# GuoYi0/alphaFive

Hardware: AMD Instinct MI355X
Metric: self-play moves/sec (11x11, 500 sims/move) (higher is better)
Workload: dtype f32 (fp16x2 split operands: 3 fp16 MFMA products per MAC, fp32 accumulate)

## Files before the change

alphafive_amd/csrc/af_engine.hip:

```cpp

#include <hip/hip_runtime.h>
#include <stdint.h>
#include <stdio.h>
#include <stdlib.h>
#include <string.h>

#include <type_traits>
#include <vector>

#include "af_engine.h"
#include "af_noise.h"

typedef unsigned long long u64;

enum { PH_IDLE = 0, PH_MOVE_START = 1, PH_SEARCH = 2, PH_MOVE_DONE = 3, PH_ERROR = 4, PH_DESCENT = 5  };
enum { CT_SIMS = 0, CT_SELECTS, CT_EXPANDS, CT_TERMINALS, CT_PLIES, CT_EPISODES, CT_LSUM, CT_LEXP,
       CT_GC, CT_GC_SCANNED, CT_YIELDS, CT_STALLS, CT_N };
enum { HIST_WORK = 0, HIST_TIME = 64, HIST_MAXTIME = 96, HIST_N = 97 };

struct EngineParams {
    int G, S, C, goal, sims, upper, training, mode, node_cap, max_ply, budget, budget_hard;
    uint32_t hash_mask;
    double init_temp, tau_decay, tau_decay_r, alpha, c_puct;
    float c_puct32;
    uint32_t k0, seed_hi, first_game_id;
    u64 colmask[4], boardmask[4];
    int32_t *phase, *pending, *sims_left, *ply, *root_last, *nodes, *nfree, *depth, *leaf_last, *leaf_slot, *status, *random_a;
    int32_t *action, *has_policy, *visits;
    float* policy;
    u64 *root, *leaf;
    double* tau;
    uint32_t *episode, *sel, *plyctr;
    int32_t *path_node, *path_cell;
    uint32_t* hash;
    u64* node_key;
    int32_t* node_sum;
    int32_t* free_idx;
    int32_t* edge_n;
    float *edge_w, *edge_p;
    int32_t* edge_c;
    double* edge_w64;
    int32_t w64;
    uint32_t *ep_seq, *ep_popped;
    int32_t* ep_len;
    float* ep_final;
    u64* rec_key;
    float* rec_policy;
    int32_t *rec_visits, *rec_last, *rec_action;
    u64* counters;
    u64* progress;
    u64* hist;
    u64* memo_key;
    float* memo_pv;
    float* memo_val;
    u64* memo_lock;
    u64* memo_stats;
    uint32_t memo_bucket_mask;
    int memo_max_stones;
    uint32_t memo_epoch;
    int memo_budget;
};
enum { MEMO_SERIAL = 0, MEMO_PROBES, MEMO_HITS, MEMO_INSERTS, MEMO_REPLACED, MEMO_N };

__device__ __forceinline__ uint32_t rfl32(uint32_t x) { return (uint32_t)__builtin_amdgcn_readfirstlane((int)x); }
__device__ __forceinline__ int rfli(int x) { return __builtin_amdgcn_readfirstlane(x); }
__device__ __forceinline__ u64 rfl64(u64 x) {
    return ((u64)rfl32((uint32_t)(x >> 32)) << 32) | (u64)rfl32((uint32_t)x);
}
__device__ __forceinline__ float rflf(float x) { return __int_as_float(rfli(__float_as_int(x))); }
template <int CTRL, int ROWS = 0xF>
__device__ __forceinline__ int dpp_i(int v) { return __builtin_amdgcn_update_dpp(v, v, CTRL, ROWS, 0xF, false); }
__device__ __forceinline__ int wave_max_i32(int v) {
    int o;
    o = dpp_i<0xB1>(v); v = o > v ? o : v;
    o = dpp_i<0x4E>(v); v = o > v ? o : v;
    o = dpp_i<0x141>(v); v = o > v ? o : v;
    o = dpp_i<0x140>(v); v = o > v ? o : v;
    o = dpp_i<0x142, 0xA>(v); v = o > v ? o : v;
    o = dpp_i<0x143, 0xC>(v); v = o > v ? o : v;
    return __builtin_amdgcn_readlane(v, 63);
}
__device__ __forceinline__ float wave_max_f32(float v) {
    float o;
    o = __int_as_float(dpp_i<0xB1>(__float_as_int(v))); v = o > v ? o : v;
    o = __int_as_float(dpp_i<0x4E>(__float_as_int(v))); v = o > v ? o : v;
    o = __int_as_float(dpp_i<0x141>(__float_as_int(v))); v = o > v ? o : v;
    o = __int_as_float(dpp_i<0x140>(__float_as_int(v))); v = o > v ? o : v;
    o = __int_as_float(dpp_i<0x142, 0xA>(__float_as_int(v))); v = o > v ? o : v;
    o = __int_as_float(dpp_i<0x143, 0xC>(__float_as_int(v))); v = o > v ? o : v;
    return __int_as_float(__builtin_amdgcn_readlane(__float_as_int(v), 63));
}


template <int CTRL>
__device__ __forceinline__ double dpp_f64(double v) {
    const int lo = __double2loint(v), hi = __double2hiint(v);
    return __hiloint2double(__builtin_amdgcn_update_dpp(hi, hi, CTRL, 0xF, 0xF, false), __builtin_amdgcn_update_dpp(lo, lo, CTRL, 0xF, 0xF, false));
}
__device__ __forceinline__ double wave_sum_f64_tree(double acc) {
    {
        const int lo = __double2loint(acc), hi = __double2hiint(acc);
        const auto a = __builtin_amdgcn_permlane32_swap(lo, lo, false, false), b = __builtin_amdgcn_permlane32_swap(hi, hi, false, false);
        acc = __hiloint2double(b[0], a[0]) + __hiloint2double(b[1], a[1]);
    }
    {
        const int lo = __double2loint(acc), hi = __double2hiint(acc);
        const auto a = __builtin_amdgcn_permlane16_swap(lo, lo, false, false), b = __builtin_amdgcn_permlane16_swap(hi, hi, false, false);
        acc = __hiloint2double(b[0], a[0]) + __hiloint2double(b[1], a[1]);
    }
    acc = acc + dpp_f64<0x128>(acc);
    acc = acc + dpp_f64<0x124>(acc);
    acc = acc + dpp_f64<0x4E>(acc);
    acc = acc + dpp_f64<0xB1>(acc);
// ... 199 lines not shown
    return h & P.memo_bucket_mask;
}
template <int KW>
__device__ __forceinline__ u64 memo_word(const EngineParams& P, const u64* mine, const u64* theirs, int last, int w) {
    const u64 kw = key_word<KW>(mine, theirs, w);
    return w == 2 * KW ? (((u64)P.memo_epoch << 32) | (u64)(uint32_t)(last + 1)) : kw;
}
template <int KW>
__device__ __forceinline__ int memo_probe(const EngineParams& P, uint32_t bucket, const u64* mine, const u64* theirs, int last, int lane,
                                          uint32_t* empty_ways) {
    constexpr int MK = 4 * KW;
    const int w = lane & (MK - 1);
    const u64 expect = memo_word<KW>(P, mine, theirs, last, w);
    u64 have = expect;
    if (lane < 4 * MK) have = P.memo_key[(size_t)bucket * (4 * MK) + lane];
    const u64 bad = __ballot(have != expect);
    const u64 blank = __ballot(lane < 4 * MK && w == 2 * KW && (uint32_t)(have >> 32) != P.memo_epoch);
    uint32_t em = 0;
    int hit = -1;
#pragma unroll
    for (int v = 3; v >= 0; --v) {
        const u64 wm = (MK == 16 ? 0xffffull : 0xffull) << (v * MK);
        if ((bad & wm) == 0ull) hit = (int)bucket * 4 + v;
        if (blank & wm) em |= 1u << v;
    }
    *empty_ways = em;
    return hit;
}


__device__ float pairwise_block(const float* a, int n) {
    if (n < 8) {
        float r = 0.0f;
        for (int i = 0; i < n; ++i) r = r + a[i];
        return r;
    }
    float r0 = a[0], r1 = a[1], r2 = a[2], r3 = a[3], r4 = a[4], r5 = a[5], r6 = a[6], r7 = a[7];
    int i;
    for (i = 8; i < n - (n % 8); i += 8) {
        r0 = r0 + a[i]; r1 = r1 + a[i + 1]; r2 = r2 + a[i + 2]; r3 = r3 + a[i + 3];
        r4 = r4 + a[i + 4]; r5 = r5 + a[i + 5]; r6 = r6 + a[i + 6]; r7 = r7 + a[i + 7];
    }
    float res = ((r0 + r1) + (r2 + r3)) + ((r4 + r5) + (r6 + r7));
    for (; i < n; ++i) res = res + a[i];
    return res;
}
__device__ float pairwise_sum(const float* a, int n) {
    if (n <= 128) return pairwise_block(a, n);
    int n2 = n / 2;
    n2 -= n2 % 8;
    return pairwise_block(a, n2) + pairwise_block(a + n2, n - n2);
}

#ifndef AF_TICK_MIN_WAVES
#define AF_TICK_MIN_WAVES 4
#endif
#ifdef AF_TICK_TIMING
__device__ unsigned long long g_tick_cycles[8192][13];
#define TK_T(var) const unsigned long long var = __builtin_readcyclecounter()
#define TK_ACC(slot, a, b) tk[slot] += (b) - (a)
#else
#define TK_T(var)
#define TK_ACC(slot, a, b)
#endif

template <int KW, bool W64, bool MEMO = false>
__global__ __launch_bounds__(64, AF_TICK_MIN_WAVES) void af_tick_kernel(EngineParams P, const float* __restrict__ policy_in,
                                                     const float* __restrict__ value_in, float* __restrict__ planes_out) {
    constexpr int CP = 64 * KW;
    __shared__ float s_pv[CP];
    __shared__ double s_cdf[CP];
    const int g = blockIdx.x;
    const int lane = threadIdx.x;
    const int C = P.C, NCAP = P.node_cap;
    if constexpr (MEMO) {
        if (g == 0 && lane == 0) atomicAdd(reinterpret_cast<unsigned long long*>(&P.memo_stats[MEMO_SERIAL]), 1ull);
    }

    int phase = rfli(P.phase[g]);
    if (phase == PH_IDLE || phase == PH_MOVE_DONE || phase == PH_ERROR) return;
    const u64 t_start = wall_clock64();
#ifdef AF_TICK_TIMING
    unsigned long long tk[13] = {0, 0, 0, 0, 0, 0, 0, 0, 0, 0, 0, 0, 0};
#endif
    TK_T(tk_entry);

    u64 root_m[KW], root_t[KW];
#pragma unroll
    for (int k = 0; k < KW; ++k) {
        root_m[k] = rfl64(P.root[(size_t)g * 2 * KW + k]);
        root_t[k] = rfl64(P.root[(size_t)g * 2 * KW + KW + k]);
    }
    int root_last = rfli(P.root_last[g]);
    int sims_left = rfli(P.sims_left[g]);
    int ply = rfli(P.ply[g]);
    int nodes = rfli(P.nodes[g]);
    int nfree = rfli(P.nfree[g]);
    double tau = P.tau[g];
    uint32_t episode = rfl32(P.episode[g]);
    uint32_t sel = rfl32(P.sel[g]);
    uint32_t plyctr = rfl32(P.plyctr[g]);
    const int random_a = rfli(P.random_a[g]);
    const uint32_t inv_s16 = (65536u + (uint32_t)P.S - 1u) / (uint32_t)P.S;
    const uint32_t k0 = P.k0, k1 = P.seed_hi + (P.first_game_id + (uint32_t)g);
    uint32_t ct[CT_N];
#pragma unroll
    for (int i = 0; i < CT_N; ++i) ct[i] = 0;
    int err = 0;

    u64* const nkeys = P.node_key + (size_t)g * NCAP * (2 * KW);
    int32_t* const nsum = P.node_sum + (size_t)g * NCAP;
    int32_t* const fre = P.free_idx + (size_t)g * NCAP;
    int32_t* const en = P.edge_n + (size_t)g * NCAP * CP;
    constexpr bool w64 = W64;
    float* const ew = P.edge_w + (w64 ? (size_t)0 : (size_t)g * NCAP * CP);
    double* const ew64 = P.edge_w64 + (w64 ? (size_t)g * NCAP * CP : (size_t)0);
    float* const ep = P.edge_p + (size_t)g * NCAP * CP;
    int32_t* const ec = P.edge_c + (size_t)g * NCAP * CP;
    uint32_t* const slots = P.hash + (size_t)g * (P.hash_mask + 1);
    int32_t* const pnode = P.path_node + (size_t)g * CP;
    int32_t* const pcell = P.path_cell + (size_t)g * CP;

    auto backup = [&](int depth, float v, int is_f32) {
        for (int d = lane; d < depth; d += 64) {
            const size_t off = (size_t)pnode[d] * CP + pcell[d];
            const float vv = ((depth - d) & 1) ? -v : v;
            const int32_t raw = en[off];
            if (w64) {
                en[off] = raw + 1;
                ew64[off] = ew64[off] + (double)vv;
            } else {
                en[off] = (raw + 1) | (is_f32 ? (int32_t)0x80000000 : 0);
                ew[off] = ew[off] + vv;
            }
        }
        __syncthreads();
    };

    TK_T(tk_loaded);
    TK_ACC(0, tk_entry, tk_loaded);
    u64 lm[KW], lt[KW];
    int c_depth = 0;
    uint32_t c_slot = 0;
    const float* c_pol = policy_in + (size_t)g * C;
    const float* c_val = value_in + g;
    bool have_eval = rfli(P.pending[g]) != 0;
    if (have_eval) {
#pragma unroll
        for (int k = 0; k < KW; ++k) {
            lm[k] = rfl64(P.leaf[(size_t)g * 2 * KW + k]);
            lt[k] = rfl64(P.leaf[(size_t)g * 2 * KW + KW + k]);
        }
        c_depth = rfli(P.depth[g]);
        c_slot = rfl32((uint32_t)P.leaf_slot[g]);
    }
    int status = AF_STATUS_IDLE;
    bool parked = false;
    int work = 0;
    uint32_t memo_probes = 0, memo_hits = 0;
  for (;;) {
    if (have_eval) {
        have_eval = false;
        u64 legal[KW];
#pragma unroll
        for (int k = 0; k < KW; ++k) legal[k] = ~(lm[k] | lt[k]) & P.boardmask[k];
        const int depth = c_depth;
        const uint32_t slot = c_slot;
        float pk[KW];
#pragma unroll
        for (int k = 0; k < KW; ++k) {
            const int c = lane + 64 * k;
            pk[k] = ((legal[k] >> lane) & 1ull) ? c_pol[c] : 0.0f;
        }
#pragma unroll
        for (int k = 0; k < KW; ++k) s_pv[lane + 64 * k] = pk[k];
        __syncthreads();
        float s = 0.0f;
#pragma unroll
        for (int i = 0; i < CP; i += 4) {
            const float4 v4 = *reinterpret_cast<const float4*>(&s_pv[i]);
            s = s + v4.x; s = s + v4.y; s = s + v4.z; s = s + v4.w;
        }
        s = rflf(s);
        if (!((double)s >= 1e-5)) s = (float)1e-5;
        if ((nfree == 0 && nodes >= NCAP) || slot == 0xffffffffu) {
            err = AF_ERR_NODE_CAP;
        } else {
            int idx;
            if (nfree > 0) idx = rfli(fre[--nfree]); else idx = nodes++;
            if (lane < 2 * KW) nkeys[(size_t)idx * 2 * KW + lane] = key_word<KW>(lm, lt, lane);
            if (lane == 0) {
                nsum[idx] = 0; slots[slot] = (uint32_t)idx + 1u;
                if (depth > 0) ec[(size_t)pnode[depth - 1] * CP + pcell[depth - 1]] = idx + 1;
            }
#pragma unroll
            for (int k = 0; k < KW; ++k) {
                const size_t off = (size_t)idx * CP + lane + 64 * k;
                en[off] = 0;
                ec[off] = 0;
                if (w64) ew64[off] = 0.0; else ew[off] = 0.0f;
                ep[off] = ((legal[k] >> lane) & 1ull) ? pk[k] / s : 0.0f;
            }
            __syncthreads();
            backup(depth, rflf(*c_val), 1);
            ct[CT_EXPANDS]++;
            ct[CT_LEXP] += (uint32_t)bb_count<KW>(legal);
        }
        ct[CT_SIMS]++;
        sims_left--;
    }

    TK_T(tk_consumed);
    TK_ACC(1, tk_loaded, tk_consumed);
    while (!parked && !err && !(MEMO && have_eval)) {
        TK_T(tk_iter);
        if (work >= ((MEMO && memo_hits) ? P.memo_budget : P.budget) && phase != PH_DESCENT) { status = AF_STATUS_YIELD; parked = true; ct[CT_YIELDS]++; break; }
        if (phase == PH_MOVE_START) {
            if (P.mode == AF_MODE_SELFPLAY && ply == 0 && rfl32(P.ep_seq[g]) - rfl32(P.ep_popped[g]) >= 2u) {
                status = AF_STATUS_YIELD; parked = true; ct[CT_STALLS]++;
                break;
            }
            bool collected = false;
            if (nodes - nfree + P.sims + 2 > NCAP && nodes > 0) {
                for (uint32_t s_ = lane; s_ <= P.hash_mask; s_ += 64) slots[s_] = 0;
                __syncthreads();
                const int rc = bb_count<KW>(root_m) + bb_count<KW>(root_t);
                int nf = 0;
                for (int base = 0; base < nodes; base += 64) {
                    const int i = base + lane;
                    const bool valid = i < nodes;
                    bool keep = false;
                    if (valid && nsum[i] >= 0) {
                        u64 nm[KW], nt[KW];
#pragma unroll
                        for (int k = 0; k < KW; ++k) { nm[k] = nkeys[(size_t)i * 2 * KW + k]; nt[k] = nkeys[(size_t)i * 2 * KW + KW + k]; }
                        const int nc = bb_count<KW>(nm) + bb_count<KW>(nt);
                        keep = true;
#pragma unroll
                        for (int k = 0; k < KW; ++k) {
                            const u64 a = ((nc ^ rc) & 1) ? nt[k] : nm[k];
                            const u64 b = ((nc ^ rc) & 1) ? nm[k] : nt[k];
                            keep = keep && ((a & root_m[k]) == root_m[k]) && ((b & root_t[k]) == root_t[k]);
                        }
                        if (keep) {
                            uint32_t h = key_hash<KW>(nm, nt);
                            for (;;) {
                                h &= P.hash_mask;
                                if (atomicCAS(&slots[h], 0u, (uint32_t)i + 1u) == 0u) break;
                                ++h;
                            }
                        } else {
                            nsum[i] = -1;
                        }
                    }
                    const u64 dm = __ballot(valid && !keep);
                    if (valid && !keep) fre[nf + __popcll(dm & ((1ull << lane) - 1ull))] = i;
                    nf += __popcll(dm);
                }
                nfree = nf;
                __syncthreads();
                __threadfence();
                ct[CT_GC]++; ct[CT_GC_SCANNED] += (uint32_t)nodes;
                collected = true;
            }
            uint32_t slot;
            const int ridx = tree_lookup<KW>(P, g, root_m, root_t, lane, &slot);
// ... 88 lines not shown
            }
#pragma unroll
            for (int k = 0; k < KW; ++k) {
                P.policy[(size_t)g * CP + lane + 64 * k] = pol[k];
                P.visits[(size_t)g * CP + lane + 64 * k] = nv[k] < 0 ? 0 : nv[k];
            }
            if (lane == 0) { P.action[g] = action; P.has_policy[g] = has_policy; }

            if (P.mode == AF_MODE_EXTERNAL) {
                phase = PH_MOVE_DONE;
                status = AF_STATUS_MOVE_DONE;
                parked = true;
                break;
            }
            if (ply >= P.max_ply) { err = AF_ERR_STATE; break; }
            const uint32_t seq = rfl32(P.ep_seq[g]);
            const size_t rslot = ((size_t)g * 2 + (seq & 1u)) * P.max_ply + ply;
            if (lane < 2 * KW) P.rec_key[rslot * 2 * KW + lane] = key_word<KW>(root_m, root_t, lane);
#pragma unroll
            for (int k = 0; k < KW; ++k) {
                const int c = lane + 64 * k;
                if (c < C) { P.rec_policy[rslot * C + c] = pol[k]; P.rec_visits[rslot * C + c] = nv[k] < 0 ? 0 : nv[k]; }
            }
            if (lane == 0) { P.rec_last[rslot] = root_last; P.rec_action[rslot] = action; }
            {
                u64 nm[KW], nt[KW];
#pragma unroll
                for (int k = 0; k < KW; ++k) { nm[k] = root_t[k]; nt[k] = root_m[k]; }
                bb_set<KW>(nt, action);
#pragma unroll
                for (int k = 0; k < KW; ++k) { root_m[k] = nm[k]; root_t[k] = nt[k]; }
            }
            root_last = action;
            ++ply;
            float fv;
            if (terminal_test<KW>(P, root_m, root_t, &fv)) {
                if (seq - rfl32(P.ep_popped[g]) >= 2u) { err = AF_ERR_EP_OVERRUN; break; }
                if (lane == 0) {
                    P.ep_len[(size_t)g * 2 + (seq & 1u)] = ply;
                    P.ep_final[(size_t)g * 2 + (seq & 1u)] = fv;
                    P.ep_seq[g] = seq + 1u;
                }
                ct[CT_EPISODES]++;
                if (lane == 0) atomicAdd(&P.progress[1], 1ull);
                for (uint32_t s_ = lane; s_ <= P.hash_mask; s_ += 64) slots[s_] = 0;
                __syncthreads();
                nodes = 0; nfree = 0;
#pragma unroll
                for (int k = 0; k < KW; ++k) { root_m[k] = 0; root_t[k] = 0; }
                root_last = -1;
                ply = 0;
                tau = P.init_temp;
                episode += 1; sel = 0; plyctr = 0;
            }
            phase = PH_MOVE_START;
            continue;
        }

        TK_T(tk_sim);
        TK_ACC(2, tk_iter, tk_sim);
        u64 cm[KW], ctb[KW];
        int last, depth;
        if (phase == PH_DESCENT) {
#pragma unroll
            for (int k = 0; k < KW; ++k) {
                cm[k] = rfl64(P.leaf[(size_t)g * 2 * KW + k]);
                ctb[k] = rfl64(P.leaf[(size_t)g * 2 * KW + KW + k]);
            }
            last = rfli(P.leaf_last[g]); depth = rfli(P.depth[g]);
            phase = PH_SEARCH;
        } else {
#pragma unroll
            for (int k = 0; k < KW; ++k) { cm[k] = root_m[k]; ctb[k] = root_t[k]; }
            last = root_last; depth = 0;
        }
        int hint = 0, pidx = -1, pcl = 0;
        typedef typename std::conditional<W64, double, float>::type wrow_t;
        int32_t r_raw[KW], r_c[KW];
        float r_p[KW];
        wrow_t r_w[KW];
        int32_t r_sum = 0;
        bool r_have = false;
        for (;;) {
            TK_T(tk_a);
            float tv;
            bool term;
            if (depth == 0)
                term = P.mode == AF_MODE_EXTERNAL ? (bool)terminal_test<KW, false>(P, cm, ctb, &tv) : false;
            else
                term = (depth > 0 && P.goal <= 8) ? (bool)terminal_through_last<KW>(P, cm, ctb, last, inv_s16, lane, &tv)
                                                                       : (bool)terminal_test<KW, true>(P, cm, ctb, &tv);
            if (term) {
                backup(depth, tv, 0);
                ct[CT_TERMINALS]++; ct[CT_SIMS]++;
                sims_left--;
                break;
            }
            uint32_t slot = 0xffffffffu;
            int idx;
            if (hint) {
                idx = hint - 1;
            } else {
                idx = tree_lookup<KW>(P, g, cm, ctb, lane, &slot);
                if (idx >= 0 && pidx >= 0 && lane == 0) ec[(size_t)pidx * CP + pcl] = idx + 1;
            }
            if (idx < 0) {
                if constexpr (MEMO) {
                    if (slot != 0xffffffffu && bb_count<KW>(cm) + bb_count<KW>(ctb) <= P.memo_max_stones) {
                        uint32_t unused;
                        const int me = memo_probe<KW>(P, memo_bucket<KW>(P, cm, ctb, last), cm, ctb, last, lane, &unused);
                        ++memo_probes;
                        if (me >= 0) {
                            ++memo_hits;
#pragma unroll
                            for (int k = 0; k < KW; ++k) { lm[k] = cm[k]; lt[k] = ctb[k]; }
                            c_depth = depth; c_slot = slot;
                            c_pol = P.memo_pv + (size_t)me * CP;
                            c_val = P.memo_val + me;
                            have_eval = true;
                            break;
                        }
                    }
                }
                if (lane < 2 * KW) P.leaf[(size_t)g * 2 * KW + lane] = key_word<KW>(cm, ctb, lane);
                if (lane == 0) { P.depth[g] = depth; P.leaf_last[g] = last; P.leaf_slot[g] = (int32_t)slot; }
                float* out = planes_out + (size_t)g * 3 * C;
#pragma unroll
                for (int k = 0; k < KW; ++k) {
                    const int c = lane + 64 * k;
                    if (c < C) {
                        out[c] = ((cm[k] >> lane) & 1ull) ? 1.0f : 0.0f;
                        out[C + c] = ((ctb[k] >> lane) & 1ull) ? 1.0f : 0.0f;
                        out[2 * C + c] = c == last ? 1.0f : 0.0f;
                    }
                }
                status = AF_STATUS_NEED_EVAL;
                parked = true;
                break;
            }
            if (work >= P.budget_hard) {
                if (lane < 2 * KW) P.leaf[(size_t)g * 2 * KW + lane] = key_word<KW>(cm, ctb, lane);
                if (lane == 0) { P.depth[g] = depth; P.leaf_last[g] = last; }
                phase = PH_DESCENT; status = AF_STATUS_YIELD; parked = true; ct[CT_YIELDS]++;
                break;
            }
            TK_T(tk_b);
            TK_ACC(3, tk_a, tk_b);
            const bool is_root = depth == 0;
            u64 legal[KW];
#pragma unroll
            for (int k = 0; k < KW; ++k) legal[k] = ~(cm[k] | ctb[k]) & P.boardmask[k];
            if (!r_have) {
                r_sum = nsum[idx];
#pragma unroll
                for (int k = 0; k < KW; ++k) {
                    const size_t off = (size_t)idx * CP + lane + 64 * k;
                    r_raw[k] = en[off];
                    r_c[k] = ec[off];
                    if constexpr (W64) r_w[k] = ew64[off]; else r_w[k] = ew[off];
                    r_p[k] = ep[off];
                }
            }
            r_have = false;
            const int sum_n = rfli(r_sum) + 1;
            if (lane == 0) nsum[idx] = sum_n;
            const uint32_t sel_id = sel++;
            int nn[KW];
            float pp[KW];
            wrow_t ww[KW];
            bool ff[KW];
            int32_t cc[KW];
#pragma unroll
            for (int k = 0; k < KW; ++k) {
                nn[k] = r_raw[k] & 0x7fffffff;
                ff[k] = r_raw[k] < 0;
                cc[k] = r_c[k];
                ww[k] = r_w[k];
                pp[k] = r_p[k];
            }
            double dd[KW];
            if (P.training) {
#ifdef AF_TICK_TIMING
                int tk_myit = 0;
#endif
                {
                    const float a_ = (float)P.alpha, inv_a = 1.0f / a_, one_m_a = 1.0f - a_;
                    uint32_t todo = 0;
#pragma unroll
                    for (int k = 0; k < KW; ++k) { dd[k] = 0.0; todo |= ((legal[k] >> lane) & 1ull) ? (1u << k) : 0u; }
                    af_u32x4 rk[KW];
                    uint32_t pend = 0;
#pragma unroll
                    for (int k = 0; k < KW; ++k) {
                        rk[k] = af_philox4x32(sel_id, episode, (AF_STREAM_GAMMA << 24) | (uint32_t)(lane + 64 * k), 0u, k0, k1);
                        float X;
                        const int ok = af_gamma_round(a_, inv_a, one_m_a, rk[k].v[0], rk[k].v[1], &X);
                        const bool lg = (todo >> k) & 1u;
                        dd[k] = (lg && ok) ? (double)X : 0.0;
                        pend |= (lg && !ok) ? (1u << k) : 0u;
                        if (KW > 2 && (k & 1)) __builtin_amdgcn_sched_barrier(0);
                    }
#ifdef AF_TICK_TIMING
                    ++tk_myit;
#endif
                    todo = pend;
                    {
                    uint32_t it = 1;
                    af_u32x4 r = rk[0];
#pragma unroll
                    for (int q = 1; q < KW; ++q) if (!(todo & ((1u << q) - 1u))) r = rk[q];
                    while (todo) {
#ifdef AF_TICK_TIMING
                        ++tk_myit;
#endif
                        const int k = __builtin_ctz(todo);
                        if ((it & 1u) == 0u) r = af_philox4x32(sel_id, episode, (AF_STREAM_GAMMA << 24) | (uint32_t)(lane + 64 * k), it >> 1, k0, k1);
                        const uint32_t wu = (it & 1u) ? r.v[2] : r.v[0], wv = (it & 1u) ? r.v[3] : r.v[1];
                        float X;
                        const int ok = af_gamma_round(a_, inv_a, one_m_a, wu, wv, &X);
                        if (ok || it == 0xFFFFu) {
                            const double Xd = ok ? (double)X : 0.0;
#pragma unroll
                            for (int q = 0; q < KW; ++q) dd[q] = q == k ? Xd : dd[q];
                            todo &= todo - 1u;
                            it = 1;
#pragma unroll
                            for (int q = 1; q < KW; ++q) if (todo && !(todo & ((1u << q) - 1u))) r = rk[q];
                        } else {
                            ++it;
                        }
                    }
                    }
                }
#ifdef AF_TICK_TIMING
                tk[12] += (unsigned long long)wave_max_i32(tk_myit);
#endif
                TK_T(tk_n1);
                TK_ACC(8, tk_b, tk_n1);
                double acc = 0.0;
#pragma unroll
                for (int k = 0; k < KW; ++k) acc = k == 0 ? dd[0] : acc + dd[k];
                acc = wave_sum_f64_tree(acc);
                if (acc == 0.0) {
                    int cnt = 0;
#pragma unroll
                    for (int k = 0; k < KW; ++k) cnt += __popcll(legal[k]);
                    const double u = 1.0 / (double)cnt;
#pragma unroll
                    for (int k = 0; k < KW; ++k) dd[k] = ((legal[k] >> lane) & 1ull) ? u : 0.0;
                } else {
                    const double inv = 1.0 / acc;
#pragma unroll
                    for (int k = 0; k < KW; ++k) dd[k] = dd[k] * inv;
                }
                TK_T(tk_n1e);
                TK_ACC(9, tk_n1, tk_n1e);
            }
            TK_T(tk_n2);
            const double sq = sqrt((double)(sum_n + 1));
            float sc[KW];
            float mx = -3.0e38f;
#pragma unroll
            for (int k = 0; k < KW; ++k) {
                const bool lg = (legal[k] >> lane) & 1ull;
                double q64;
                if (nn[k] == 0) q64 = 0.0;
                else if (!W64 && ff[k]) q64 = (double)((float)ww[k] / (float)nn[k]);
                else q64 = (double)ww[k] / (double)nn[k];
                double t;
                if (P.training) {
                    double p_;
                    if (is_root) p_ = (double)(0.75f * pp[k]) + 0.25 * dd[k];
                    else p_ = (double)(0.9f * pp[k]) + 0.1 * dd[k];
                    t = ((P.c_puct * p_) * sq) / (double)(1 + nn[k]);
                } else {
                    t = ((double)(P.c_puct32 * pp[k]) * sq) / (double)(1 + nn[k]);
                }
                sc[k] = lg ? (float)(q64 + t) : -3.0e38f;
                mx = sc[k] > mx ? sc[k] : mx;
            }
            TK_T(tk_n3);
            TK_ACC(10, tk_n2, tk_n3);
            int cell = -1;
            if (is_root && P.training) {
                u64 cand[KW];
#pragma unroll
                for (int k = 0; k < KW; ++k) cand[k] = __ballot(((legal[k] >> lane) & 1ull) && nn[k] == 0);
                int m = bb_count<KW>(cand);
                if (m == 0) {
#pragma unroll
                    for (int k = 0; k < KW; ++k) cand[k] = __ballot(((legal[k] >> lane) & 1ull) && nn[k] == 1);
                    m = bb_count<KW>(cand);
                }
                if (m > 0) cell = bb_select_wave<KW>(cand, (int)af_pick((uint32_t)m, sel_id, episode, AF_STREAM_PICK, k0, k1), lane);
            }
            if (cell < 0) {
                mx = wave_max_f32(mx);
                u64 cand[KW];
#pragma unroll
                for (int k = 0; k < KW; ++k) cand[k] = __ballot(((legal[k] >> lane) & 1ull) && sc[k] == mx);
                const int m = bb_count<KW>(cand);
                cell = bb_select_wave<KW>(cand, (int)af_pick((uint32_t)m, sel_id, episode, AF_STREAM_PICK, k0, k1), lane);
            }
            cell = rfli(cell);
            hint = 0;
#pragma unroll
            for (int k = 0; k < KW; ++k) { const int t_ = __builtin_amdgcn_readlane(cc[k], cell & 63); if ((cell >> 6) == k) hint = t_; }
            hint = rfli(hint);
            pidx = idx; pcl = cell;
            if (hint) {
                const int ci = hint - 1;
                r_sum = nsum[ci];
#pragma unroll
                for (int k = 0; k < KW; ++k) {
                    const size_t off = (size_t)ci * CP + lane + 64 * k;
                    r_raw[k] = en[off];
                    r_c[k] = ec[off];
                    if constexpr (W64) r_w[k] = ew64[off]; else r_w[k] = ew[off];
                    r_p[k] = ep[off];
                }
                r_have = true;
            }
            ++work;
            ct[CT_SELECTS]++;
            ct[CT_LSUM] += (uint32_t)bb_count<KW>(legal);
            if (lane == 0) { pnode[depth] = idx; pcell[depth] = cell; }
            ++depth;
            {
                u64 nm[KW], nt[KW];
#pragma unroll
                for (int k = 0; k < KW; ++k) { nm[k] = ctb[k]; nt[k] = cm[k]; }
                bb_set<KW>(nt, cell);
#pragma unroll
                for (int k = 0; k < KW; ++k) { cm[k] = nm[k]; ctb[k] = nt[k]; }
            }
            last = cell;
            __syncthreads();
            TK_T(tk_c);
            TK_ACC(4, tk_b, tk_c);
            TK_ACC(11, tk_n3, tk_c);
#ifdef AF_TICK_TIMING
            tk[7] += 1;
#endif
        }
    }
    if (!MEMO || !have_eval) break;
  }
    TK_T(tk_parked);
    if constexpr (MEMO) {
        if (lane == 0 && memo_probes) {
            atomicAdd(reinterpret_cast<unsigned long long*>(&P.memo_stats[MEMO_PROBES]), (unsigned long long)memo_probes);
            if (memo_hits) atomicAdd(reinterpret_cast<unsigned long long*>(&P.memo_stats[MEMO_HITS]), (unsigned long long)memo_hits);
        }
    }

    if (err) { phase = PH_ERROR; status = err; }
    if (lane < 2 * KW) P.root[(size_t)g * 2 * KW + lane] = key_word<KW>(root_m, root_t, lane);
    if (lane == 0) {
        P.phase[g] = phase;
        P.pending[g] = status == AF_STATUS_NEED_EVAL ? 1 : 0;
        P.root_last[g] = root_last;
        P.sims_left[g] = sims_left;
        P.ply[g] = ply;
        P.nodes[g] = nodes;
        P.nfree[g] = nfree;
        P.tau[g] = tau;
        P.episode[g] = episode;
        P.sel[g] = sel;
        P.plyctr[g] = plyctr;
        P.status[g] = status;
        for (int i = 0; i < CT_N; ++i)
            if (ct[i]) atomicAdd(reinterpret_cast<unsigned long long*>(&P.counters[(size_t)g * CT_N + i]), (unsigned long long)ct[i]);
        const u64 dt = wall_clock64() - t_start;
        atomicAdd(&P.hist[HIST_WORK + (work < 63 ? work : 63)], 1ull);
        const u64 tb = dt / 800ull;
        atomicAdd(&P.hist[HIST_TIME + (tb < 31ull ? tb : 31ull)], 1ull);
        atomicMax(&P.hist[HIST_MAXTIME], dt);
    }
#ifdef AF_TICK_TIMING
    {
        TK_T(tk_end);
        tk[5] = tk_end - tk_parked;
        tk[6] = tk_end - tk_entry;
        if (lane == 0 && g < 8192) for (int q = 0; q < 13; ++q) g_tick_cycles[g][q] = tk[q];
    }
#endif
}

__global__ __launch_bounds__(1024) void af_pack_scan(EngineParams P, int max_eps, int max_plies, int32_t* __restrict__ out) {
    __shared__ int s_e[1024], s_p[1024];
    __shared__ int s_cut;
    const int t = threadIdx.x;
    int base_e = 0, base_p = 0;
    int32_t* meta = out + 4;
    int32_t* fin = out + 4 + (size_t)max_eps * 4;
    if (t == 0) s_cut = 0x7fffffff;
    __syncthreads();
    for (int g0 = 0; g0 < P.G; g0 += 1024) {
        const int g = g0 + t;
        int ne = 0, T0 = 0, T1 = 0;
        uint32_t pop = 0;
        if (g < P.G) {
            pop = P.ep_popped[g];
            ne = (int)(P.ep_seq[g] - pop);
            if (ne >= 1) T0 = P.ep_len[(size_t)g * 2 + (pop & 1u)];
            if (ne >= 2) T1 = P.ep_len[(size_t)g * 2 + ((pop + 1u) & 1u)];
        }
        s_e[t] = ne; s_p[t] = T0 + T1;
        __syncthreads();
        for (int off = 1; off < 1024; off <<= 1) {
            const int ve = t >= off ? s_e[t - off] : 0, vp = t >= off ? s_p[t - off] : 0;
            __syncthreads();
            s_e[t] += ve; s_p[t] += vp;
            __syncthreads();
        }
        const int e_excl = base_e + s_e[t] - ne, p_excl = base_p + s_p[t] - (T0 + T1);
        int fit = 0;
        if (ne >= 1 && e_excl + 1 <= max_eps && p_excl + T0 <= max_plies) {
            fit = 1;
            if (ne >= 2 && e_excl + 2 <= max_eps && p_excl + T0 + T1 <= max_plies) fit = 2;
        }
        if (g < P.G && fit < ne) atomicMin(&s_cut, g);
        __syncthreads();
        const int cut = s_cut;
        if (g < P.G && g <= cut && fit > 0) {
            for (int k = 0; k < fit; ++k) {
                const uint32_t seq = pop + (uint32_t)k;
                const int idx = e_excl + k;
                meta[idx * 4 + 0] = g; meta[idx * 4 + 1] = (int32_t)seq;
                meta[idx * 4 + 2] = k == 0 ? T0 : T1; meta[idx * 4 + 3] = p_excl + (k == 0 ? 0 : T0);
                fin[idx] = __float_as_int(P.ep_final[(size_t)g * 2 + (seq & 1u)]);
            }
            P.ep_popped[g] = pop + (uint32_t)fit;
        }
        __syncthreads();
        if (cut != 0x7fffffff) {
            if (g == cut) {
// ... 151 lines not shown
        case AF_ERR_STATE: return "engine state error";
        default: return "unknown error";
    }
}

int af_engine_create(const af_config* cfg, int32_t num_games, int32_t device, int32_t mode, int32_t training,
                     uint64_t seed, uint32_t first_game_id, int32_t node_cap, af_engine** out) {
    if (!cfg || !out || num_games < 1) return AF_ERR_ARG;
    const int S = cfg->board_size, C = S * S;
    if (S < 2 || C > 256 || cfg->goal < 2 || cfg->goal > S || cfg->simulation_per_step < 1) return AF_ERR_ARG;
    const int value_f64 = (mode & AF_MODE_VALUE_F64) ? 1 : 0;
    mode &= ~AF_MODE_VALUE_F64;
    if (mode != AF_MODE_SELFPLAY && mode != AF_MODE_EXTERNAL) return AF_ERR_ARG;
    if (!(cfg->dirichlet_alpha > 0.0 && cfg->dirichlet_alpha < 1.0)) return AF_ERR_ARG;
    if (cfg->upper_simulation_per_step < 1 || !(cfg->c_puct >= 0.0)) return AF_ERR_ARG;
    HIP_OK(hipSetDevice(device));
    af_engine* e = new af_engine();
    e->device = device;
    e->KW = C <= 128 ? 2 : 4;
    const int KW = e->KW, CP = 64 * KW;
    EngineParams& P = e->P;
    memset(&P, 0, sizeof(P));
    P.G = num_games; P.S = S; P.C = C; P.goal = cfg->goal;
    P.sims = cfg->simulation_per_step; P.upper = cfg->upper_simulation_per_step;
    P.training = training ? 1 : 0; P.mode = mode; P.max_ply = C; P.w64 = value_f64;
    P.budget = AF_DEFAULT_TICK_BUDGET; P.budget_hard = AF_DEFAULT_TICK_BUDGET_HARD;
    if (const char* b = getenv("AF_TICK_BUDGET")) { const int v = atoi(b); if (v > 0) P.budget = v; }
    if (const char* b = getenv("AF_TICK_BUDGET_HARD")) { const int v = atoi(b); if (v > 0) P.budget_hard = v; }
    if (P.budget_hard < P.budget) P.budget_hard = P.budget;
    if (node_cap <= 0) node_cap = mode == AF_MODE_SELFPLAY ? 4 * P.sims + 64 : 32768;
    if (node_cap < P.sims + 8) node_cap = P.sims + 8;
    P.node_cap = node_cap;
    uint32_t hcap = 64;
    while (hcap < 2u * (uint32_t)node_cap) hcap <<= 1;
    P.hash_mask = hcap - 1;
    P.init_temp = cfg->init_temp; P.tau_decay = cfg->tau_decay_rate; P.tau_decay_r = cfg->tau_decay_rate_r;
    P.alpha = cfg->dirichlet_alpha; P.c_puct = cfg->c_puct; P.c_puct32 = (float)cfg->c_puct;
    P.k0 = af_key0(seed); P.seed_hi = (uint32_t)(seed >> 32); P.first_game_id = first_game_id;
    for (int c = 0; c < C; ++c) {
        P.boardmask[c >> 6] |= 1ull << (c & 63);
        if (c % S <= S - cfg->goal) P.colmask[c >> 6] |= 1ull << (c & 63);
    }
    const size_t G = num_games;
    int rc = AF_OK;
#define A(p, n) if (rc == AF_OK) rc = dalloc(e, &P.p, (n))
    A(phase, G); A(pending, G); A(sims_left, G); A(ply, G); A(root_last, G); A(nodes, G); A(nfree, G); A(depth, G);
    A(leaf_last, G); A(leaf_slot, G); A(status, G); A(random_a, G); A(action, G); A(has_policy, G);
    A(visits, G * CP); A(policy, G * CP); A(root, G * 2 * KW); A(leaf, G * 2 * KW); A(tau, G);
    A(episode, G); A(sel, G); A(plyctr, G); A(path_node, G * CP); A(path_cell, G * CP);
    A(hash, G * hcap); A(node_key, G * node_cap * 2 * KW); A(node_sum, G * node_cap); A(free_idx, G * node_cap);
    A(edge_n, G * node_cap * CP); A(edge_p, G * node_cap * CP); A(edge_c, G * node_cap * CP);
    if (value_f64) { A(edge_w64, G * node_cap * CP); A(edge_w, 64); } else { A(edge_w, G * node_cap * CP); A(edge_w64, 8); }
    A(ep_seq, G); A(ep_popped, G); A(counters, G * CT_N); A(progress, 2); A(hist, HIST_N);
    if (mode == AF_MODE_SELFPLAY) {
        const size_t R = G * 2 * P.max_ply;
        A(ep_len, G * 2); A(ep_final, G * 2); A(rec_key, R * 2 * KW); A(rec_policy, R * C); A(rec_visits, R * C);
        A(rec_last, R); A(rec_action, R);
    }
#undef A
    if (rc != AF_OK) { af_engine_destroy(e); return rc; }
    std::vector<int32_t> ph(G, mode == AF_MODE_SELFPLAY ? PH_MOVE_START : PH_IDLE), rl(G, -1);
    std::vector<double> tau(G, cfg->init_temp);
    HIP_OK(hipMemcpy(P.phase, ph.data(), G * 4, hipMemcpyHostToDevice));
    HIP_OK(hipMemcpy(P.root_last, rl.data(), G * 4, hipMemcpyHostToDevice));
    HIP_OK(hipMemcpy(P.tau, tau.data(), G * 8, hipMemcpyHostToDevice));
    e->h_i32.resize(G); e->h_i32b.resize(G); e->h_ct.resize(G * CT_N);
    *out = e;
    return AF_OK;
}

void af_engine_destroy(af_engine* e) {
    if (!e) return;
    (void)hipSetDevice(e->device);
    for (void* p : e->allocs) (void)hipFree(p);
    if (e->pack_dev) (void)hipFree(e->pack_dev);
    if (e->stage_dev) (void)hipFree(e->stage_dev);
    delete e;
}

int32_t af_engine_num_games(const af_engine* e) { return e->P.G; }
int32_t af_engine_cells(const af_engine* e) { return e->P.C; }
int32_t af_engine_key_words(const af_engine* e) { return 2 * e->KW; }
int32_t af_engine_max_plies(const af_engine* e) { return e->P.max_ply; }

int af_engine_tick(af_engine* e, void* stream, const float* policy_dev, const float* value_dev, float* planes_dev) {
    if (!e || !planes_dev) return AF_ERR_ARG;
    hipStream_t st = (hipStream_t)stream;
#define AF_TICK(KW_, W_, M_) hipLaunchKernelGGL((af_tick_kernel<KW_, W_, M_>), dim3(e->P.G), dim3(64), 0, st, e->P, policy_dev, value_dev, planes_dev)
    if (e->memo) {
        if (e->KW == 2) { if (e->P.w64) AF_TICK(2, true, true); else AF_TICK(2, false, true); }
        else { if (e->P.w64) AF_TICK(4, true, true); else AF_TICK(4, false, true); }
    } else {
        if (e->KW == 2) { if (e->P.w64) AF_TICK(2, true, false); else AF_TICK(2, false, false); }
        else { if (e->P.w64) AF_TICK(4, true, false); else AF_TICK(4, false, false); }
    }
#undef AF_TICK
    HIP_OK(hipGetLastError());
    return AF_OK;
}

int af_engine_memo_enable(af_engine* e, int32_t log2_buckets, int32_t max_stones) {
    if (!e || e->memo || log2_buckets < 4 || log2_buckets > 28 || max_stones < 0) return AF_ERR_ARG;
    HIP_OK(hipSetDevice(e->device));
    EngineParams& P = e->P;
    const size_t NE = (size_t)4 << log2_buckets, CP = 64 * (size_t)e->KW, MK = 4 * (size_t)e->KW;
    int rc = AF_OK;
    if (rc == AF_OK) rc = dalloc(e, &P.memo_key, NE * MK);
    if (rc == AF_OK) rc = dalloc(e, &P.memo_pv, NE * CP);
    if (rc == AF_OK) rc = dalloc(e, &P.memo_val, NE);
    if (rc == AF_OK) rc = dalloc(e, &P.memo_lock, NE);
    if (rc == AF_OK) rc = dalloc(e, &P.memo_stats, (size_t)MEMO_N);
    if (rc != AF_OK) return rc;
    P.memo_bucket_mask = (uint32_t)((1ull << log2_buckets) - 1ull);
    P.memo_max_stones = max_stones;
    P.memo_epoch = 1;
    P.memo_budget = P.budget < 6 ? P.budget : 6;
    if (const char* b = getenv("AF_MEMO_BUDGET")) { const int v = atoi(b); if (v > 0) { P.memo_budget = v; e->memo_budget_fixed = true; } }
    e->memo_entries = NE;
// ... 412 lines not shown
            if (i >= S || j >= S) return AF_ERR_ARG;
            const int c = i * S + j;
            key[(ch == '3' ? 0 : KW) + (c >> 6)] |= 1ull << (c & 63);
            ++j;
        } else return AF_ERR_ARG;
    }
    return AF_OK;
}

int af_engine_tree_w64(af_engine* e, int32_t game, int32_t cap, double* w) {
    if (!e || game < 0 || game >= e->P.G || !e->P.w64) return AF_ERR_ARG;
    EngineParams& P = e->P;
    const int CP = 64 * e->KW, C = P.C;
    HIP_OK(hipDeviceSynchronize());
    int32_t hw;
    HIP_OK(hipMemcpy(&hw, P.nodes + game, 4, hipMemcpyDeviceToHost));
    const size_t nb = (size_t)game * P.node_cap;
    std::vector<int32_t> bs((size_t)(hw > 0 ? hw : 1));
    if (hw > 0) HIP_OK(hipMemcpy(bs.data(), P.node_sum + nb, (size_t)hw * 4, hipMemcpyDeviceToHost));
    int live = 0;
    for (int i = 0; i < hw; ++i) live += bs[i] >= 0;
    if (cap < live || live == 0 || !w) return live;
    std::vector<double> bd((size_t)hw * CP);
    HIP_OK(hipMemcpy(bd.data(), P.edge_w64 + nb * CP, (size_t)hw * CP * 8, hipMemcpyDeviceToHost));
    int o = 0;
    for (int i = 0; i < hw; ++i) {
        if (bs[i] < 0) continue;
        for (int c = 0; c < C; ++c) w[(size_t)o * C + c] = bd[(size_t)i * CP + c];
        ++o;
    }
    return live;
}

int af_engine_set_tree_w64(af_engine* e, int32_t game, int32_t count, const double* w) {
    if (!e || game < 0 || game >= e->P.G || !e->P.w64 || e->P.mode != AF_MODE_EXTERNAL || count < 0 || count > e->P.node_cap || (count > 0 && !w))
        return AF_ERR_ARG;
    EngineParams& P = e->P;
    const int CP = 64 * e->KW, C = P.C;
    HIP_OK(hipDeviceSynchronize());
    int32_t hw;
    HIP_OK(hipMemcpy(&hw, P.nodes + game, 4, hipMemcpyDeviceToHost));
    if (hw != count) return AF_ERR_STATE;
    if (count == 0) return AF_OK;
    std::vector<double> bd((size_t)count * CP, 0.0);
    for (int i = 0; i < count; ++i)
        for (int c = 0; c < C; ++c) bd[(size_t)i * CP + c] = w[(size_t)i * C + c];
    HIP_OK(hipMemcpy(P.edge_w64 + (size_t)game * P.node_cap * CP, bd.data(), bd.size() * 8, hipMemcpyHostToDevice));
    return AF_OK;
}

#ifdef AF_TICK_TIMING
int af_engine_debug_tick_cycles(unsigned long long* host) {
    HIP_OK(hipDeviceSynchronize());
    HIP_OK(hipMemcpyFromSymbol(host, HIP_SYMBOL(g_tick_cycles), sizeof(unsigned long long) * 8192 * 13));
    return AF_OK;
}
#endif

int af_key_to_state(const uint64_t* key, int32_t S, char* out, int32_t cap) {
    if (!key || !out || S < 1 || S * S > 256) return AF_ERR_ARG;
    const int KW = S * S <= 128 ? 2 : 4;
    int n = 0;
    for (int i = 0; i < S; ++i) {
        int run = 0;
        for (int j = 0; j < S; ++j) {
            const int c = i * S + j;
            const bool m = (key[c >> 6] >> (c & 63)) & 1ull, t = (key[KW + (c >> 6)] >> (c & 63)) & 1ull;
            if (!m && !t) { ++run; continue; }
            if (run) { if (n + 1 >= cap) return AF_ERR_ARG; out[n++] = (char)('a' + run); run = 0; }
            if (n + 1 >= cap) return AF_ERR_ARG;
            out[n++] = m ? '3' : '1';
        }
        if (run) { if (n + 1 >= cap) return AF_ERR_ARG; out[n++] = (char)('a' + run); }
        if (n + 1 >= cap) return AF_ERR_ARG;
        out[n++] = '/';
    }
    out[n] = 0;
    return n;
}

}
```

Baseline: 6060.

## Precompute Dirichlet gamma noise into a per-game ring buffer ahead of selections

```diff
diff --git a/alphafive_amd/csrc/af_engine.hip b/alphafive_amd/csrc/af_engine.hip
--- a/alphafive_amd/csrc/af_engine.hip
+++ b/alphafive_amd/csrc/af_engine.hip
@@ -59,6 +59,8 @@
     int memo_max_stones;
     uint32_t memo_epoch;
     int memo_budget;
+    float* ring;
+    u64* ring_tag;
 };
 enum { MEMO_SERIAL = 0, MEMO_PROBES, MEMO_HITS, MEMO_INSERTS, MEMO_REPLACED, MEMO_N };
 
@@ -364,16 +366,89 @@
     return pairwise_block(a, n2) + pairwise_block(a + n2, n - n2);
 }
 
+#ifndef AF_RING_K
+#define AF_RING_K 16
+#endif
+#ifndef AF_RING_J
+#define AF_RING_J 2
+#endif
+static_assert((AF_RING_K & (AF_RING_K - 1)) == 0 && AF_RING_K >= 2 && AF_RING_K <= 64, "AF_RING_K: a power of two, one tag per lane");
+
+template <int KW, int J>
+__device__ __forceinline__ void ring_fill(const EngineParams& P, float* __restrict__ ring_g, u64* __restrict__ tag_g, const uint32_t (&ids)[J],
+                                          uint32_t episode, uint32_t k0, uint32_t k1, int lane) {
+    constexpr int CP = 64 * KW, N = J * KW;
+    const float a_ = (float)P.alpha, inv_a = 1.0f / a_, one_m_a = 1.0f - a_;
+    af_u32x4 rk[N];
+    float x[N];
+    uint32_t todo = 0;
+#pragma unroll
+    for (int q = 0; q < N; ++q) {
+        const int i = q / KW, k = q % KW;
+        rk[q] = af_philox4x32(ids[i], episode, (AF_STREAM_GAMMA << 24) | (uint32_t)(lane + 64 * k), 0u, k0, k1);
+        float X;
+        const int ok = af_gamma_round(a_, inv_a, one_m_a, rk[q].v[0], rk[q].v[1], &X);
+        const bool on = (P.boardmask[k] >> lane) & 1ull;
+        x[q] = (on && ok) ? X : 0.0f;
+        todo |= (on && !ok) ? (1u << q) : 0u;
+    }
+    uint32_t it = 1;
+    af_u32x4 r = rk[0];
+#pragma unroll
+    for (int q = 1; q < N; ++q) if (!(todo & ((1u << q) - 1u))) r = rk[q];
+    while (todo) {
+        const int q0 = __builtin_ctz(todo);
+        if ((it & 1u) == 0u) {
+            uint32_t id = ids[0];
+#pragma unroll
+            for (int i = 1; i < J; ++i) id = (q0 / KW) == i ? ids[i] : id;
+            r = af_philox4x32(id, episode, (AF_STREAM_GAMMA << 24) | (uint32_t)(lane + 64 * (q0 % KW)), it >> 1, k0, k1);
+        }
+        const uint32_t wu = (it & 1u) ? r.v[2] : r.v[0], wv = (it & 1u) ? r.v[3] : r.v[1];
+        float X;
+        const int ok = af_gamma_round(a_, inv_a, one_m_a, wu, wv, &X);
+        if (ok || it == 0xFFFFu) {
+            const float Xf = ok ? X : 0.0f;
+#pragma unroll
+            for (int q = 0; q < N; ++q) x[q] = q == q0 ? Xf : x[q];
+            todo &= todo - 1u;
+            it = 1;
+#pragma unroll
+            for (int q = 1; q < N; ++q) if (todo && !(todo & ((1u << q) - 1u))) r = rk[q];
+        } else {
+            ++it;
+        }
+    }
+#pragma unroll
+    for (int q = 0; q < N; ++q) {
+        const int i = q / KW, k = q % KW;
+        ring_g[(size_t)(ids[i] & (AF_RING_K - 1)) * CP + lane + 64 * k] = x[q];
+    }
+#pragma unroll
+    for (int i = 0; i < J; ++i)
+        if (lane == i) tag_g[ids[i] & (AF_RING_K - 1)] = ((u64)episode << 32) | (u64)ids[i];
+}
+
 #ifndef AF_TICK_MIN_WAVES
 #define AF_TICK_MIN_WAVES 4
 #endif
 #ifdef AF_TICK_TIMING
-__device__ unsigned long long g_tick_cycles[8192][13];
+__device__ unsigned long long g_tick_cycles[8192][14];
 #define TK_T(var) const unsigned long long var = __builtin_readcyclecounter()
 #define TK_ACC(slot, a, b) tk[slot] += (b) - (a)
+#define TK_MARK(var) unsigned long long var = __builtin_readcyclecounter()
+#define TK_PHASE(slot, mark) do { const unsigned long long n_ = __builtin_readcyclecounter(); tk[slot] += n_ - (mark); (mark) = n_; } while (0)
 #else
 #define TK_T(var)
 #define TK_ACC(slot, a, b)
+#define TK_MARK(var)
+#define TK_PHASE(slot, mark)
+#endif
+#ifdef AF_TICK_CONST_NOISE
+#define AF_TICK_RING 0
+#endif
+#ifndef AF_TICK_RING
+#define AF_TICK_RING 1
 #endif
 
 template <int KW, bool W64, bool MEMO = false>
@@ -393,7 +468,7 @@
     if (phase == PH_IDLE || phase == PH_MOVE_DONE || phase == PH_ERROR) return;
     const u64 t_start = wall_clock64();
 #ifdef AF_TICK_TIMING
-    unsigned long long tk[13] = {0, 0, 0, 0, 0, 0, 0, 0, 0, 0, 0, 0, 0};
+    unsigned long long tk[14] = {0, 0, 0, 0, 0, 0, 0, 0, 0, 0, 0, 0, 0, 0};
 #endif
     TK_T(tk_entry);
 
@@ -451,6 +526,36 @@
 
     TK_T(tk_loaded);
     TK_ACC(0, tk_entry, tk_loaded);
+    float* const ring_g = P.ring + (size_t)g * AF_RING_K * CP;
+    const bool ring_on = AF_TICK_RING && P.training && P.ring != nullptr;
+    int ring_left = ring_on ? AF_RING_K : 0;
+    auto ring_refill = [&](uint32_t episode, uint32_t sel) {
+        u64* const tag_g = P.ring_tag + (size_t)g * AF_RING_K;
+        const uint32_t my_id = sel + (uint32_t)lane;
+        u64 miss = __ballot(lane < AF_RING_K && tag_g[my_id & (AF_RING_K - 1)] != (((u64)episode << 32) | (u64)my_id));
+        constexpr int RJ = KW == 2 ? AF_RING_J : 1;
+        while (miss) {
+            uint32_t ids[RJ];
+            int n = 0;
+#pragma unroll
+            for (int i = 0; i < RJ; ++i) {
+                if (miss) { ids[i] = sel + (uint32_t)__builtin_ctzll(miss); miss &= miss - 1ull; ++n; } else ids[i] = ids[0];
+            }
+            if (n == RJ) {
+                ring_fill<KW, RJ>(P, ring_g, tag_g, ids, episode, k0, k1, lane);
+            } else {
+                for (int i = 0; i < n; ++i) {
+                    uint32_t one[1] = {ids[0]};
+#pragma unroll
+                    for (int q = 1; q < RJ; ++q) one[0] = i == q ? ids[q] : one[0];
+                    ring_fill<KW, 1>(P, ring_g, tag_g, one, episode, k0, k1, lane);
+                }
+            }
+        }
+    };
+    if (ring_on) ring_refill(episode, sel);
+    TK_T(tk_ringed);
+    TK_ACC(13, tk_loaded, tk_ringed);
     u64 lm[KW], lt[KW];
     int c_depth = 0;
     uint32_t c_slot = 0;
@@ -523,7 +628,7 @@
     }
 
     TK_T(tk_consumed);
-    TK_ACC(1, tk_loaded, tk_consumed);
+    TK_ACC(1, tk_ringed, tk_consumed);
     while (!parked && !err && !(MEMO && have_eval)) {
         TK_T(tk_iter);
         if (work >= ((MEMO && memo_hits) ? P.memo_budget : P.budget) && phase != PH_DESCENT) { status = AF_STATUS_YIELD; parked = true; ct[CT_YIELDS]++; break; }
@@ -718,6 +823,7 @@
                 ply = 0;
                 tau = P.init_temp;
                 episode += 1; sel = 0; plyctr = 0;
+                ring_left = 0;
             }
             phase = PH_MOVE_START;
             continue;
@@ -745,6 +851,7 @@
         int32_t r_raw[KW], r_c[KW];
         float r_p[KW];
         wrow_t r_w[KW];
+        float r_x[KW];
         int32_t r_sum = 0;
         bool r_have = false;
         for (;;) {
@@ -816,6 +923,9 @@
             u64 legal[KW];
 #pragma unroll
             for (int k = 0; k < KW; ++k) legal[k] = ~(cm[k] | ctb[k]) & P.boardmask[k];
+            const uint32_t sel_id = sel++;
+            const bool ringed = ring_left > 0;
+            ring_left -= ringed ? 1 : 0;
             if (!r_have) {
                 r_sum = nsum[idx];
 #pragma unroll
@@ -827,10 +937,13 @@
                     r_p[k] = ep[off];
                 }
             }
+            if (ringed && !r_have) {
+#pragma unroll
+                for (int k = 0; k < KW; ++k) r_x[k] = ring_g[(size_t)(sel_id & (AF_RING_K - 1)) * CP + lane + 64 * k];
+            }
             r_have = false;
             const int sum_n = rfli(r_sum) + 1;
             if (lane == 0) nsum[idx] = sum_n;
-            const uint32_t sel_id = sel++;
             int nn[KW];
             float pp[KW];
             wrow_t ww[KW];
@@ -844,8 +957,31 @@
                 ww[k] = r_w[k];
                 pp[k] = r_p[k];
             }
+            TK_MARK(tk_m);
+            int cell = -1;
+            if (is_root && P.training) {
+                u64 cand[KW];
+#pragma unroll
+                for (int k = 0; k < KW; ++k) cand[k] = __ballot(((legal[k] >> lane) & 1ull) && nn[k] == 0);
+                int m = bb_count<KW>(cand);
+                if (m == 0) {
+#pragma unroll
+                    for (int k = 0; k < KW; ++k) cand[k] = __ballot(((legal[k] >> lane) & 1ull) && nn[k] == 1);
+                    m = bb_count<KW>(cand);
+                }
+                if (m > 0) cell = bb_select_wave<KW>(cand, (int)af_pick((uint32_t)m, sel_id, episode, AF_STREAM_PICK, k0, k1), lane);
+            }
+            if (cell < 0) {
             double dd[KW];
             if (P.training) {
+                if (ringed) {
+#pragma unroll
+                    for (int k = 0; k < KW; ++k) dd[k] = ((legal[k] >> lane) & 1ull) ? (double)r_x[k] : 0.0;
+                } else {
+#ifdef AF_TICK_CONST_NOISE
+#pragma unroll
+                    for (int k = 0; k < KW; ++k) dd[k] = ((legal[k] >> lane) & 1ull) ? 0.5 : 0.0;
+#else
 #ifdef AF_TICK_TIMING
                 int tk_myit = 0;
 #endif
@@ -901,8 +1037,9 @@
 #ifdef AF_TICK_TIMING
                 tk[12] += (unsigned long long)wave_max_i32(tk_myit);
 #endif
-                TK_T(tk_n1);
-                TK_ACC(8, tk_b, tk_n1);
+#endif
+                }
+                TK_PHASE(8, tk_m);
                 double acc = 0.0;
 #pragma unroll
                 for (int k = 0; k < KW; ++k) acc = k == 0 ? dd[0] : acc + dd[k];
@@ -919,10 +1056,8 @@
 #pragma unroll
                     for (int k = 0; k < KW; ++k) dd[k] = dd[k] * inv;
                 }
-                TK_T(tk_n1e);
-                TK_ACC(9, tk_n1, tk_n1e);
-            }
-            TK_T(tk_n2);
+                TK_PHASE(9, tk_m);
+            }
             const double sq = sqrt((double)(sum_n + 1));
             float sc[KW];
             float mx = -3.0e38f;
@@ -945,28 +1080,15 @@
                 sc[k] = lg ? (float)(q64 + t) : -3.0e38f;
                 mx = sc[k] > mx ? sc[k] : mx;
             }
-            TK_T(tk_n3);
-            TK_ACC(10, tk_n2, tk_n3);
-            int cell = -1;
-            if (is_root && P.training) {
-                u64 cand[KW];
-#pragma unroll
-                for (int k = 0; k < KW; ++k) cand[k] = __ballot(((legal[k] >> lane) & 1ull) && nn[k] == 0);
-                int m = bb_count<KW>(cand);
-                if (m == 0) {
-#pragma unroll
-                    for (int k = 0; k < KW; ++k) cand[k] = __ballot(((legal[k] >> lane) & 1ull) && nn[k] == 1);
-                    m = bb_count<KW>(cand);
-                }
-                if (m > 0) cell = bb_select_wave<KW>(cand, (int)af_pick((uint32_t)m, sel_id, episode, AF_STREAM_PICK, k0, k1), lane);
-            }
-            if (cell < 0) {
+            TK_PHASE(10, tk_m);
+            {
                 mx = wave_max_f32(mx);
                 u64 cand[KW];
 #pragma unroll
                 for (int k = 0; k < KW; ++k) cand[k] = __ballot(((legal[k] >> lane) & 1ull) && sc[k] == mx);
                 const int m = bb_count<KW>(cand);
                 cell = bb_select_wave<KW>(cand, (int)af_pick((uint32_t)m, sel_id, episode, AF_STREAM_PICK, k0, k1), lane);
+            }
             }
             cell = rfli(cell);
             hint = 0;
@@ -984,6 +1106,7 @@
                     r_c[k] = ec[off];
                     if constexpr (W64) r_w[k] = ew64[off]; else r_w[k] = ew[off];
                     r_p[k] = ep[off];
+                    if (ring_left > 0) r_x[k] = ring_g[(size_t)(sel & (AF_RING_K - 1)) * CP + lane + 64 * k];
                 }
                 r_have = true;
             }
@@ -1004,7 +1127,7 @@
             __syncthreads();
             TK_T(tk_c);
             TK_ACC(4, tk_b, tk_c);
-            TK_ACC(11, tk_n3, tk_c);
+            TK_PHASE(11, tk_m);
 #ifdef AF_TICK_TIMING
             tk[7] += 1;
 #endif
@@ -1048,7 +1171,7 @@
         TK_T(tk_end);
         tk[5] = tk_end - tk_parked;
         tk[6] = tk_end - tk_entry;
-        if (lane == 0 && g < 8192) for (int q = 0; q < 13; ++q) g_tick_cycles[g][q] = tk[q];
+        if (lane == 0 && g < 8192) for (int q = 0; q < 14; ++q) g_tick_cycles[g][q] = tk[q];
     }
 #endif
 }
@@ -1306,6 +1429,9 @@
     A(edge_n, G * node_cap * CP); A(edge_p, G * node_cap * CP); A(edge_c, G * node_cap * CP);
     if (value_f64) { A(edge_w64, G * node_cap * CP); A(edge_w, 64); } else { A(edge_w, G * node_cap * CP); A(edge_w64, 8); }
     A(ep_seq, G); A(ep_popped, G); A(counters, G * CT_N); A(progress, 2); A(hist, HIST_N);
+    const char* ring_env = getenv("AF_NOISE_RING");
+    const bool ring = !(ring_env && atoi(ring_env) == 0);
+    if (ring) { A(ring, G * AF_RING_K * CP); A(ring_tag, G * AF_RING_K); }
     if (mode == AF_MODE_SELFPLAY) {
         const size_t R = G * 2 * P.max_ply;
         A(ep_len, G * 2); A(ep_final, G * 2); A(rec_key, R * 2 * KW); A(rec_policy, R * C); A(rec_visits, R * C);
@@ -1318,6 +1444,11 @@
     HIP_OK(hipMemcpy(P.phase, ph.data(), G * 4, hipMemcpyHostToDevice));
     HIP_OK(hipMemcpy(P.root_last, rl.data(), G * 4, hipMemcpyHostToDevice));
     HIP_OK(hipMemcpy(P.tau, tau.data(), G * 8, hipMemcpyHostToDevice));
+    if (ring) {
+        std::vector<u64> tags(G * AF_RING_K);
+        for (size_t i = 0; i < tags.size(); ++i) tags[i] = (u64)(i % AF_RING_K) + 1ull;
+        HIP_OK(hipMemcpy(P.ring_tag, tags.data(), tags.size() * 8, hipMemcpyHostToDevice));
+    }
     e->h_i32.resize(G); e->h_i32b.resize(G); e->h_ct.resize(G * CT_N);
     *out = e;
     return AF_OK;
@@ -1836,7 +1967,7 @@
 #ifdef AF_TICK_TIMING
 int af_engine_debug_tick_cycles(unsigned long long* host) {
     HIP_OK(hipDeviceSynchronize());
-    HIP_OK(hipMemcpyFromSymbol(host, HIP_SYMBOL(g_tick_cycles), sizeof(unsigned long long) * 8192 * 13));
+    HIP_OK(hipMemcpyFromSymbol(host, HIP_SYMBOL(g_tick_cycles), sizeof(unsigned long long) * 8192 * 14));
     return AF_OK;
 }
 #endif
```

After: 6101, median of 6. About the same (+0.7%).
